# FeatureBaseDB/featurebase

Measured on AMD Instinct MI355X. Metric: container set-ops/sec + bits-scanned GB/s, 1M-col Intersect+Count, higher is better.
Workload: dtype u64

## Files before the change

### featurebase_amd/csrc/fbk_fold_kernels.hip.h

```cpp
#pragma once
#include "fbk_query_kernels.hip.h"

namespace fbk {

template <int OP>
__device__ __forceinline__ void lds_acc32(uint32_t* p, uint32_t m) {
  if (OP == 2) atomicXor(p, m);
  else atomicOr(p, m);
}

template <int OP>
__device__ __forceinline__ void lds_fill32(uint32_t* p) {
  if (OP == 2) atomicXor(p, ~0u);
  else *(__attribute__((address_space(3))) uint32_t*)p = ~0u;
}

template <int OP>
__device__ __forceinline__ void scatter_chunk(const uint32_t (&d)[4], uint32_t type, uint32_t len, uint32_t j, int lane,
                                              uint32_t* acc32) {
  if (type == kTypeBitmap) {
    u64* acc64 = reinterpret_cast<u64*>(acc32);
    const uint32_t w = (j * kWave + lane) * 2;
    const u64 x = ((u64)d[1] << 32) | d[0], y = ((u64)d[3] << 32) | d[2];
    if (OP == 2) {
      atomicXor(&acc64[w], x);
      atomicXor(&acc64[w + 1], y);
    } else {
      atomicOr(&acc64[w], x);
      atomicOr(&acc64[w + 1], y);
    }
    return;
  }
  if (type == kTypeArray) {
    const uint32_t row0 = j * (kWave * 8u);
    if (row0 + kWave * 8u <= len) {
#pragma unroll
      for (int q = 0; q < 4; ++q) {
        lds_acc32<OP>(&acc32[(d[q] >> 5) & 0x7FFu], 1u << (d[q] & 31));
        lds_acc32<OP>(&acc32[d[q] >> 21], 1u << ((d[q] >> 16) & 31));
      }
    } else {
      const uint32_t e0 = row0 + lane * 8u;
      if (e0 < len) {
        const uint32_t valid = (1u << min(len - e0, 8u)) - 1u;
#pragma unroll
        for (int q = 0; q < 4; ++q) {
          lds_acc32<OP>(&acc32[(d[q] >> 5) & 0x7FFu], __builtin_amdgcn_ubfe(valid, 2u * q, 1u) << (d[q] & 31));
          lds_acc32<OP>(&acc32[d[q] >> 21], __builtin_amdgcn_ubfe(valid, 2u * q + 1u, 1u) << ((d[q] >> 16) & 31));
        }
      }
    }
    return;
  }
  const uint32_t i0 = (j * kWave + lane) * 4u;
#pragma unroll
  for (int t = 0; t < 4; ++t) {
    const bool on = i0 + t < len;
    const uint32_t s = d[t] & 0xFFFFu, l = d[t] >> 16;
    const uint32_t ws = s >> 5, we = l >> 5;
    const uint32_t ms = ~0u << (s & 31), ml = ~0u >> (31 - (l & 31));
    if (on) {
      if (ws == we) {
        lds_acc32<OP>(&acc32[ws], ms & ml);
      } else {
        lds_acc32<OP>(&acc32[ws], ms);
        lds_acc32<OP>(&acc32[we], ml);
      }
    }
    const uint32_t inner = (on && we > ws + 1) ? we - ws - 1 : 0;
    if (inner && inner <= 4)
      for (uint32_t q = ws + 1; q < we; ++q) lds_fill32<OP>(&acc32[q]);
    u64 longm = __ballot(inner > 4);
    while (longm) {
      const int src = __builtin_ctzll(longm);
      longm &= longm - 1;
      const uint32_t bs = __builtin_amdgcn_readlane(ws, src), be = __builtin_amdgcn_readlane(we, src);
      for (uint32_t q = bs + 1 + lane; q < be; q += kWave) lds_fill32<OP>(&acc32[q]);
    }
  }
}

template <int OP>
__device__ __forceinline__ void scatter_big(const uint8_t* __restrict__ p, uint32_t type, uint32_t len, int lane,
                                            uint32_t* acc32) {
  if (type == kTypeArray) {
    const uint16_t* q = reinterpret_cast<const uint16_t*>(p);
    for (uint32_t i = lane; i < len; i += kWave) {
      const uint32_t a = q[i];
      lds_acc32<OP>(&acc32[a >> 5], 1u << (a & 31));
    }
  } else {
    const uint32_t* q = reinterpret_cast<const uint32_t*>(p);
    for (uint32_t i = lane; i < len; i += kWave) {
      const uint32_t iv = q[i], s = iv & 0xFFFFu, l = iv >> 16;
      const uint32_t ws = s >> 5, we = l >> 5;
      const uint32_t ms = ~0u << (s & 31), ml = ~0u >> (31 - (l & 31));
      if (ws == we) {
        lds_acc32<OP>(&acc32[ws], ms & ml);
      } else {
        lds_acc32<OP>(&acc32[ws], ms);
        lds_acc32<OP>(&acc32[we], ml);
        for (uint32_t d = ws + 1; d < we; ++d) lds_acc32<OP>(&acc32[d], ~0u);
      }
    }
  }
}

template <int OP, int WRITE>
__global__ void __launch_bounds__(256, 8) k_fold_scatter(const Slot* __restrict__ slots, const uint8_t* __restrict__ arena,
                                                     const uint32_t* __restrict__ rows, uint64_t n_groups, uint32_t k,
                                                     const Slot* __restrict__ fslots, const uint8_t* __restrict__ farena,
                                                     const uint32_t* __restrict__ frows, uint8_t* __restrict__ arenaO,
                                                     Slot* __restrict__ outSlots, uint32_t* __restrict__ outRuns,
                                                     u64* __restrict__ out_counts, const Slot* __restrict__ recs) {
  static_assert(OP == 1 || OP == 2 || OP == 3, "scatter fold handles OR, XOR and ANDNOT");
  __shared__ u64 acc[kWords];
  __shared__ u64 aux[kWords];
  __shared__ uint32_t s_short;
  __shared__ uint32_t s_cnt[3][4];
  __shared__ uint32_t s_scan[2][4];
  const int t = threadIdx.x;
  const int lane = t & 63;
  const int wv = __builtin_amdgcn_readfirstlane(t >> 6);
  const uint64_t cell = xcd_swizzle(blockIdx.x, gridDim.x);
  const uint64_t g = cell >> 4;
  const uint32_t slot = cell & 15;
  if (g >= n_groups) return;
  uint32_t* acc32 = reinterpret_cast<uint32_t*>(acc);
  {
    ulonglong2 z;
    z.x = z.y = 0;
    reinterpret_cast<ulonglong2*>(acc)[t] = z;
    reinterpret_cast<ulonglong2*>(acc)[256 + t] = z;
    if (t == 0) s_short = 0;
  }
  __syncthreads();
  const uint32_t* grow = rows + g * k;
  const Slot* grec = recs ? recs + cell * (uint64_t)k : nullptr;
  Slot sf;
  sf.off = 0;
  sf.len = 0;
  sf.tn = 0;
  u64 pf[4] = {0, 0, 0, 0};
  bool f_ready = false;
  if (fslots) {
    sf = fslots[(uint64_t)frows[g] * kSlots + slot];
    if (slot_n(sf) != 0 && slot_type(sf) == kTypeBitmap) {
      const ulonglong2* q = reinterpret_cast<const ulonglong2*>(farena + sf.off);
      const ulonglong2 v0 = ld_stream(&q[t]), v1 = ld_stream(&q[256 + t]);
      pf[0] = v0.x;
      pf[1] = v0.y;
      pf[2] = v1.x;
      pf[3] = v1.y;
      f_ready = true;
    }
  }
  Slot s0;
  s0.off = 0;
  s0.len = 0;
  s0.tn = 0;
  u64 p0[4] = {0, 0, 0, 0};
  bool r0_ready = false;
  if (OP == 3) {
    s0 = grec ? grec[0] : slots[(uint64_t)grow[0] * kSlots + slot];
    if (slot_n(s0) != 0 && slot_type(s0) == kTypeBitmap) {
      const ulonglong2* q = reinterpret_cast<const ulonglong2*>(arena + s0.off);
      const ulonglong2 v0 = ld_stream(&q[t]), v1 = ld_stream(&q[256 + t]);
      p0[0] = v0.x;
      p0[1] = v0.y;
      p0[2] = v1.x;
      p0[3] = v1.y;
      r0_ready = true;
    }
  }
  bool shortcut = false;
  for (uint32_t base = 0; base < k && !shortcut; base += 64) {
    Slot mine;
    mine.off = 0;
    mine.len = 0;
    mine.tn = 0;
    if (base + lane < k) mine = grec ? grec[base + lane] : slots[(uint64_t)grow[base + lane] * kSlots + slot];
    if (OP == 3 && base + lane == 0) mine.tn = 0;
    const uint32_t cnt = min(64u, k - base);
    if (OP != 2 && __ballot(slot_n(mine) == 65536u) != 0) {
      shortcut = true;
      break;
    }
    auto meta = [&](uint32_t i, u64& off, uint32_t& len, uint32_t& tn) {
      const uint32_t lo = __builtin_amdgcn_readlane((uint32_t)mine.off, (int)(i & 63));
      const uint32_t hi = __builtin_amdgcn_readlane((uint32_t)(mine.off >> 32), (int)(i & 63));
      off = ((u64)hi << 32) | lo;
      len = __builtin_amdgcn_readlane(mine.len, (int)(i & 63));
      tn = __builtin_amdgcn_readlane(mine.tn, (int)(i & 63));
    };
    {
      u64 bigm = __ballot((mine.tn & 0xFFFFFFu) != 0 && payload_bytes(mine.tn >> 24, mine.len) > 8192u);
      for (uint32_t ord = 0; bigm; ++ord) {
        const uint32_t i = (uint32_t)__builtin_ctzll(bigm);
        bigm &= bigm - 1;
        if ((ord & 3u) == (uint32_t)wv) {
          u64 off;
          uint32_t len, tn;
          meta(i, off, len, tn);
          scatter_big<OP>(arena + off, tn >> 24, len, lane, acc32);
        }
      }
    }
    {
      constexpr int NCH = 6;
      typedef uint32_t Chunk __attribute__((ext_vector_type(4)));
      Chunk C[NCH];
      const uint32_t my_bytes = payload_bytes(mine.tn >> 24, mine.len);
      const uint32_t nr = ((mine.tn & 0xFFFFFFu) != 0 && my_bytes <= 8192u) ? (my_bytes + 1023u) >> 10 : 0u;
      auto next_valid = [&](uint32_t i) {
        while (i < cnt && __builtin_amdgcn_readlane(nr, (int)(i & 63)) == 0) i += 4;
        return i;
      };
      struct Cursor {
        uint32_t i, j, nr, len, tn, bytes;
        u64 off;
      };
      auto fetch = [&](Cursor& k) {
        k.j = 0;
        if (k.i < cnt) {
          meta(k.i, k.off, k.len, k.tn);
          k.bytes = payload_bytes(k.tn >> 24, k.len);
          k.nr = (k.bytes + 1023u) >> 10;
        }
      };
      auto advance = [&](Cursor& k) {
        if (++k.j == k.nr) {
          k.i = next_valid(k.i + 4);
          fetch(k);
        }
      };
      Cursor P, Q;
      P.i = next_valid(wv);
      P.nr = P.len = P.tn = P.bytes = 0;
      P.off = 0;
      fetch(P);
      Q = P;
      const uint32_t lane16 = lane * 16u;
      auto load_chunk = [&](Chunk& c) {
        const uint8_t* p = arena;
        if (P.i < cnt) {
          const uint32_t b0 = P.j * 1024u + lane16;
          p = arena + P.off + (b0 < P.bytes ? b0 : 0u);
          advance(P);
        }
        asm volatile("global_load_dwordx4 %0, %1, off nt" : "=&v"(c) : "v"(p));
      };
#pragma unroll
      for (int q = 0; q < NCH; ++q) load_chunk(C[q]);
      while (Q.i < cnt) {
#pragma unroll
        for (int q = 0; q < NCH; ++q) {
          asm volatile("s_waitcnt vmcnt(%1)" : "+v"(C[q]) : "n"(NCH - 1));
          if (Q.i < cnt) {
            const uint32_t d[4] = {C[q][0], C[q][1], C[q][2], C[q][3]};
            scatter_chunk<OP>(d, Q.tn >> 24, Q.len, Q.j, lane, acc32);
            advance(Q);
          }
          load_chunk(C[q]);
        }
      }
      asm volatile("s_waitcnt vmcnt(0)" ::: "memory");
    }
  }
  if (shortcut && lane == 0) s_short = 1;
  __syncthreads();
  const bool sat = s_short != 0;

  u64 w[4];
  {
    const ulonglong2 v0 = reinterpret_cast<const ulonglong2*>(acc)[t], v1 = reinterpret_cast<const ulonglong2*>(acc)[256 + t];
    w[0] = sat ? ~0ull : v0.x;
    w[1] = sat ? ~0ull : v0.y;
    w[2] = sat ? ~0ull : v1.x;
    w[3] = sat ? ~0ull : v1.y;
  }
  auto load_block = [&](const Slot& s, const uint8_t* __restrict__ ar, u64 (&o)[4]) {
    if (slot_n(s) == 0) {
      o[0] = o[1] = o[2] = o[3] = 0;
      return;
    }
    if (slot_type(s) == kTypeBitmap) {
      const ulonglong2* q = reinterpret_cast<const ulonglong2*>(ar + s.off);
      const ulonglong2 v0 = ld_stream(&q[t]), v1 = ld_stream(&q[256 + t]);
      o[0] = v0.x;
      o[1] = v0.y;
      o[2] = v1.x;
      o[3] = v1.y;
      return;
    }
    __syncthreads();
    if (t < kWave) {
      u64 f[kWordsPerLane];
      frag_load(s, ar, t, aux, f);
      lds_write_frag(aux, t, f);
    }
    __syncthreads();
    const ulonglong2 v0 = reinterpret_cast<const ulonglong2*>(aux)[t], v1 = reinterpret_cast<const ulonglong2*>(aux)[256 + t];
    o[0] = v0.x;
    o[1] = v0.y;
    o[2] = v1.x;
    o[3] = v1.y;
  };
  if (OP == 3) {
    if (!r0_ready) load_block(s0, arena, p0);
#pragma unroll
    for (int q = 0; q < 4; ++q) w[q] = p0[q] & ~w[q];
  }
  uint32_t cu = __popcll(w[0]) + __popcll(w[1]) + __popcll(w[2]) + __popcll(w[3]);
  uint32_t cf = cu;
  if (fslots) {
    if (!f_ready) load_block(sf, farena, pf);
    cf = __popcll(w[0] & pf[0]) + __popcll(w[1] & pf[1]) + __popcll(w[2] & pf[2]) + __popcll(w[3] & pf[3]);
  }
  uint32_t rr = 0;
  if (WRITE == 2 || (WRITE && outRuns)) {
    __syncthreads();
    {
      ulonglong2 v0, v1;
      v0.x = w[0];
      v0.y = w[1];
      v1.x = w[2];
      v1.y = w[3];
      reinterpret_cast<ulonglong2*>(aux)[t] = v0;
      reinterpret_cast<ulonglong2*>(aux)[256 + t] = v1;
    }
    __syncthreads();
    const u64 l0 = t ? (aux[2 * t - 1] >> 63) : 0ull, l1 = aux[512 + 2 * t - 1] >> 63;
    rr = __popcll(w[0] & ~((w[0] << 1) | l0)) + __popcll(w[1] & ~((w[1] << 1) | (w[0] >> 63))) +
         __popcll(w[2] & ~((w[2] << 1) | l1)) + __popcll(w[3] & ~((w[3] << 1) | (w[2] >> 63)));
  }
  cu = wave_reduce_add(cu);
  cf = wave_reduce_add(cf);
  rr = wave_reduce_add(rr);
  if (lane == 0) {
    s_cnt[0][wv] = cu;
    s_cnt[1][wv] = cf;
    s_cnt[2][wv] = rr;
  }
  __syncthreads();
  const uint32_t tot_u = s_cnt[0][0] + s_cnt[0][1] + s_cnt[0][2] + s_cnt[0][3];
  const uint32_t tot_f = s_cnt[1][0] + s_cnt[1][1] + s_cnt[1][2] + s_cnt[1][3];
  if (WRITE == 2) {
    const uint32_t tot_r = s_cnt[2][0] + s_cnt[2][1] + s_cnt[2][2] + s_cnt[2][3];
    const uint32_t enc = tot_u == 0 ? kTypeNil : (tot_r <= 2048u && tot_r <= tot_u / 2u) ? kTypeRun : tot_u < 4096u ? kTypeArray : kTypeBitmap;
    Slot so;
    so.off = enc == kTypeNil ? 0ull : cell * 8192ull;
    so.len = 0;
    so.tn = make_tn(enc, tot_u);
    uint8_t* dst = arenaO + cell * 8192ull;
    if (enc == kTypeBitmap) {
      ulonglong2* q = reinterpret_cast<ulonglong2*>(dst);
      ulonglong2 v0, v1;
      v0.x = w[0];
      v0.y = w[1];
      v1.x = w[2];
      v1.y = w[3];
      st_stream(&q[t], v0);
      st_stream(&q[256 + t], v1);
      so.len = kWords;
    } else if (enc != kTypeNil) {
      uint16_t* st16 = reinterpret_cast<uint16_t*>(acc);
      const uint32_t v0 = 128u * (uint32_t)t, v1 = 32768u + 128u * (uint32_t)t;
      u64 a0 = w[0], a1 = w[1], a2 = w[2], a3 = w[3];
      u64 e0 = 0, e1 = 0, e2 = 0, e3 = 0;
      if (enc == kTypeRun) {
        const u64 l0 = t ? (aux[2 * t - 1] >> 63) : 0ull, l1 = aux[512 + 2 * t - 1] >> 63;
        const u64 n0 = aux[2 * t + 2] & 1ull, n1 = t < 255 ? (aux[512 + 2 * t + 2] & 1ull) : 0ull;
        a0 = w[0] & ~((w[0] << 1) | l0);
        a1 = w[1] & ~((w[1] << 1) | (w[0] >> 63));
        a2 = w[2] & ~((w[2] << 1) | l1);
        a3 = w[3] & ~((w[3] << 1) | (w[2] >> 63));
        e0 = w[0] & ~((w[0] >> 1) | ((w[1] & 1ull) << 63));
        e1 = w[1] & ~((w[1] >> 1) | (n0 << 63));
        e2 = w[2] & ~((w[2] >> 1) | ((w[3] & 1ull) << 63));
        e3 = w[3] & ~((w[3] >> 1) | (n1 << 63));
      }
      const uint32_t ca = (uint32_t)(__popcll(a0) + __popcll(a1)) | ((uint32_t)(__popcll(a2) + __popcll(a3)) << 16);
      const uint32_t ce = (uint32_t)(__popcll(e0) + __popcll(e1)) | ((uint32_t)(__popcll(e2) + __popcll(e3)) << 16);
      const uint32_t ia = wave_incl_scan(ca), ie = wave_incl_scan(ce);
      if (lane == 63) {
        s_scan[0][wv] = ia;
        s_scan[1][wv] = ie;
      }
      __syncthreads();
      uint32_t wa = 0, we = 0, ta = 0, te = 0;
#pragma unroll
      for (int k = 0; k < 4; ++k) {
        if (k < wv) wa += s_scan[0][k], we += s_scan[1][k];
        ta += s_scan[0][k], te += s_scan[1][k];
      }
      const uint32_t xa = wa + ia - ca, xe = we + ie - ce;
      uint32_t pa0 = xa & 0xFFFFu, pa1 = (ta & 0xFFFFu) + (xa >> 16);
      uint32_t pe0 = xe & 0xFFFFu, pe1 = (te & 0xFFFFu) + (xe >> 16);
      const uint32_t stride = enc == kTypeRun ? 2u : 1u;
      auto emit = [&](u64 bits, uint32_t base, uint32_t& at, uint32_t odd) {
        while (bits) {
          st16[stride * (at++) + odd] = (uint16_t)(base + (uint32_t)__builtin_ctzll(bits));
          bits &= bits - 1;
        }
      };
      emit(a0, v0, pa0, 0u);
      emit(a1, v0 + 64u, pa0, 0u);
      emit(a2, v1, pa1, 0u);
      emit(a3, v1 + 64u, pa1, 0u);
      if (enc == kTypeRun) {
        emit(e0, v0, pe0, 1u);
        emit(e1, v0 + 64u, pe0, 1u);
        emit(e2, v1, pe1, 1u);
        emit(e3, v1 + 64u, pe1, 1u);
      }
      __syncthreads();
      so.len = enc == kTypeRun ? tot_r : tot_u;
      const uint32_t chunks = ((enc == kTypeRun ? 4u * tot_r : 2u * tot_u) + 15u) >> 4;
      const ulonglong2* src = reinterpret_cast<const ulonglong2*>(acc);
      ulonglong2* q = reinterpret_cast<ulonglong2*>(dst);
      if ((uint32_t)t < chunks) st_stream(&q[t], src[t]);
      if (256u + (uint32_t)t < chunks) st_stream(&q[256 + t], src[256 + t]);
    }
    if (t == 0) outSlots[cell] = so;
  } else if (WRITE) {
    Slot so;
    so.off = cell * 8192ull;
    so.len = kWords;
    so.tn = make_tn(tot_u ? kTypeBitmap : kTypeNil, tot_u);
    if (tot_u) {
      ulonglong2* q = reinterpret_cast<ulonglong2*>(arenaO + so.off);
      ulonglong2 v0, v1;
      v0.x = w[0];
      v0.y = w[1];
      v1.x = w[2];
      v1.y = w[3];
      st_stream(&q[t], v0);
      st_stream(&q[256 + t], v1);
    }
    if (t == 0) {
      outSlots[cell] = so;
      if (outRuns) outRuns[cell] = s_cnt[2][0] + s_cnt[2][1] + s_cnt[2][2] + s_cnt[2][3];
    }
  }
  if (t == 0 && tot_f && out_counts) atomicAdd(&out_counts[g], (u64)tot_f);
}

}
```

Baseline: 461.3 million.

## Hoist first slot-metadata load and defer filter bitmap load behind chunk prefetch

For OR/XOR folds, the first batch of row slot descriptors is now loaded before the accumulator is zeroed, so its latency overlaps the LDS clear and barrier. The filter bitmap load is moved after the scatter loop's initial chunk loads are issued, so the streaming payload fetch starts earlier and does not queue behind the filter load. It also adds optional compile-time wall-clock stamps per block for profiling, which are off by default. The reorder keeps the filter data in registers longer, which may raise register pressure.

```diff
diff --git a/featurebase_amd/csrc/fbk_fold_kernels.hip.h b/featurebase_amd/csrc/fbk_fold_kernels.hip.h
--- a/featurebase_amd/csrc/fbk_fold_kernels.hip.h
+++ b/featurebase_amd/csrc/fbk_fold_kernels.hip.h
@@ -2,6 +2,10 @@
 #include "fbk_query_kernels.hip.h"
 
 namespace fbk {
+
+#ifdef FBK_FOLD_STAMPS
+__device__ unsigned long long* g_fold_stamps;
+#endif
 
 template <int OP>
 __device__ __forceinline__ void lds_acc32(uint32_t* p, uint32_t m) {
@@ -126,7 +130,16 @@
   const uint64_t g = cell >> 4;
   const uint32_t slot = cell & 15;
   if (g >= n_groups) return;
+#ifdef FBK_FOLD_STAMPS
+  const unsigned long long stamp_start = wall_clock64();
+  unsigned long long stamp_primed = 0, stamp_loop = 0;
+#endif
   uint32_t* acc32 = reinterpret_cast<uint32_t*>(acc);
+  Slot first;
+  first.off = 0;
+  first.len = 0;
+  first.tn = 0;
+  if (OP != 3 && (uint32_t)lane < k) first = recs ? recs[cell * (uint64_t)k + lane] : slots[(uint64_t)rows[g * k + lane] * kSlots + slot];
   {
     ulonglong2 z;
     z.x = z.y = 0;
@@ -145,7 +158,7 @@
   bool f_ready = false;
   if (fslots) {
     sf = fslots[(uint64_t)frows[g] * kSlots + slot];
-    if (slot_n(sf) != 0 && slot_type(sf) == kTypeBitmap) {
+    if (OP == 3 && slot_n(sf) != 0 && slot_type(sf) == kTypeBitmap) {
       const ulonglong2* q = reinterpret_cast<const ulonglong2*>(farena + sf.off);
       const ulonglong2 v0 = ld_stream(&q[t]), v1 = ld_stream(&q[256 + t]);
       pf[0] = v0.x;
@@ -179,7 +192,8 @@
     mine.off = 0;
     mine.len = 0;
     mine.tn = 0;
-    if (base + lane < k) mine = grec ? grec[base + lane] : slots[(uint64_t)grow[base + lane] * kSlots + slot];
+    if ((OP == 3 || base) && base + lane < k) mine = grec ? grec[base + lane] : slots[(uint64_t)grow[base + lane] * kSlots + slot];
+    if (OP != 3 && base == 0) mine = first;
     if (OP == 3 && base + lane == 0) mine.tn = 0;
     const uint32_t cnt = min(64u, k - base);
     if (OP != 2 && __ballot(slot_n(mine) == 65536u) != 0) {
@@ -252,6 +266,20 @@
       };
 #pragma unroll
       for (int q = 0; q < NCH; ++q) load_chunk(C[q]);
+#ifdef FBK_FOLD_STAMPS
+      if (base == 0) stamp_primed = wall_clock64();
+#endif
+      if (OP != 3 && base == 0 && slot_n(sf) != 0 && slot_type(sf) == kTypeBitmap) {
+        int tt = t;
+        asm volatile("" : "+v"(tt));
+        const ulonglong2* q = reinterpret_cast<const ulonglong2*>(farena + sf.off);
+        const ulonglong2 v0 = ld_stream(&q[tt]), v1 = ld_stream(&q[256 + tt]);
+        pf[0] = v0.x;
+        pf[1] = v0.y;
+        pf[2] = v1.x;
+        pf[3] = v1.y;
+        f_ready = true;
+      }
       while (Q.i < cnt) {
 #pragma unroll
         for (int q = 0; q < NCH; ++q) {
@@ -267,9 +295,15 @@
       asm volatile("s_waitcnt vmcnt(0)" ::: "memory");
     }
   }
+#ifdef FBK_FOLD_STAMPS
+  stamp_loop = wall_clock64();
+#endif
   if (shortcut && lane == 0) s_short = 1;
   __syncthreads();
   const bool sat = s_short != 0;
+#ifdef FBK_FOLD_STAMPS
+  const unsigned long long stamp_all = wall_clock64();
+#endif
 
   u64 w[4];
   {
@@ -444,6 +478,19 @@
     }
   }
   if (t == 0 && tot_f && out_counts) atomicAdd(&out_counts[g], (u64)tot_f);
-}
-
-}
+#ifdef FBK_FOLD_STAMPS
+  if (t == 0 && g_fold_stamps) {
+    unsigned long long* st = g_fold_stamps + 8ull * cell;
+    st[0] = stamp_start;
+    st[1] = stamp_primed;
+    st[2] = stamp_loop;
+    st[3] = stamp_all;
+    st[4] = wall_clock64();
+    st[5] = (unsigned long long)__builtin_amdgcn_s_getreg(20 | (3 << 11));
+    st[6] = blockIdx.x;
+    st[7] = (unsigned long long)__builtin_amdgcn_s_getreg(4 | (31 << 11));
+  }
+#endif
+}
+
+}
```

Measured after the change: 459.4 million. No clear change (-0.4%).
